# muyeon-jo/POI_recommendation_models

Measured on NVIDIA B200. Metric: fullrank_eval_users_per_sec, higher is better.
Workload: dtype f16+e5m2-corrections/f32-accum

## Files before the change

poi_recommendation_models_b200/csrc/nais_tc.cu:

```cuda
#include <cuda_fp16.h>
#include <cuda_fp8.h>

#include <type_traits>

#include "nais_common.cuh"
#include "umma.cuh"

namespace nais {

using namespace umma;

namespace tc {

constexpr int TM = 128;
constexpr int NBUF = 3;
constexpr int ACC_STRIDE = 160;
constexpr int TPC = 3;
constexpr int EPI_WARPS = 16;
constexpr int EPI_THREADS = EPI_WARPS * 32;
constexpr int ARRIVE_WARPS = 8;
constexpr int THREADS = (EPI_WARPS + 2) * 32;
constexpr int MAX_STAGES = 4;
constexpr int SORTN = 512;
constexpr int HMETA = 512;
// ... 366 lines not shown
  const int m = (int)(room < n ? (room < 0 ? 0 : room) : n);
  return m - m % hsplit;
}

struct MainArgs {
  NaisParams p;
  NaisCatalog cat;
  NaisUsers users;
  Geo g;
  int64_t poi_begin, poi_end;
  int k, exclude, groups;
  int groups_real;
  int64_t n_items;
  const unsigned char* hdr;
  const unsigned char* Pimg;
  const unsigned char* Bimg;
  unsigned long long* part_keys;
  float* all_scores;
  const float* score_in;
  int64_t max_chunks;
  int gate;
  const int* pass_flags;
  GeoMixArgs geo;
};

__device__ __forceinline__ void epi_bar() { asm volatile("bar.sync 1, 512;" ::: "memory"); }

__device__ __forceinline__ unsigned long long warp_sort_desc(unsigned long long v, int lane) {
#pragma unroll
  for (int k = 2; k <= 32; k <<= 1) {
#pragma unroll
    for (int j = k >> 1; j > 0; j >>= 1) {
      const unsigned long long o = __shfl_xor_sync(0xffffffffu, v, j);
      const bool desc = k == 32 || (lane & k) == 0, lower = (lane & j) == 0;
      v = (lower == desc) ? (v > o ? v : o) : (v < o ? v : o);
    }
  }
  return v;
}
__device__ __forceinline__ unsigned long long warp_fold_top32(unsigned long long a, unsigned long long b, int lane) {
  const unsigned long long br = __shfl_sync(0xffffffffu, b, 31 - lane);
  unsigned long long v = a > br ? a : br;
#pragma unroll
  for (int j = 16; j > 0; j >>= 1) {
    const unsigned long long o = __shfl_xor_sync(0xffffffffu, v, j);
    v = ((lane & j) == 0) ? (v > o ? v : o) : (v < o ? v : o);
  }
  return v;
}

template <bool kSinglePart, int kHch, int kFix, int kS = 64, bool kGeo = false>
__global__ void __launch_bounds__(THREADS, 1) fullrank_tc_kernel(const __grid_constant__ MainArgs A) {
  constexpr bool kPair = kFix == 5 || kFix == 6;
  constexpr bool kFastEpi = kFix == 1 || kFix == 2 || kPair;
  constexpr bool kD128 = kFix == 3;
  static_assert(!kGeo || kFix == 0 || kFix == 4, "geo mode lives in the run-time-shape epilogue");
  constexpr int kCombA = kGeo ? 4 : 3, kCombT = (kGeo && !kSinglePart) ? 2 : TPC;
  extern __shared__ __align__(128) unsigned char smem[];
  const Geo& g = A.g;
  unsigned char* sA = smem;
  unsigned char* sB = sA + g.tpc * g.a_tile;
  unsigned char* sE = sB + g.stages * g.stage_bytes;
  unsigned char* sZ = sE + NBUF * 2 * TM * 16;
  unsigned long long* keys = reinterpret_cast<unsigned long long*>(sZ + 4096);
  float* comb = kSinglePart ? reinterpret_cast<float*>(keys + SORTN) : reinterpret_cast<float*>(sE);
  int* hm_id = reinterpret_cast<int*>(reinterpret_cast<unsigned char*>(keys + SORTN) + (kSinglePart ? 3 * kCombA * TPC * TM * 4 : 0));
  float* hm_la = reinterpret_cast<float*>(hm_id + HMETA);
  float* hm_lo = hm_la + HMETA;
  float* xch = hm_lo + HMETA;
  uint64_t* bars = reinterpret_cast<uint64_t*>(xch + 6 * TM);
  uint64_t* a_full = bars + 0;
  uint64_t* a_empty = bars + 1;
  uint64_t* b_full = bars + 2;
  uint64_t* b_empty = bars + 2 + MAX_STAGES;
  uint64_t* e_full = bars + 2 + 2 * MAX_STAGES;
  uint64_t* acc_full = e_full + NBUF;
  uint64_t* acc_empty = acc_full + 2 * NBUF;
  uint32_t* tslot = reinterpret_cast<uint32_t*>(acc_empty + NBUF);
  float* hm_cos = reinterpret_cast<float*>(reinterpret_cast<unsigned char*>(bars) + 384);
// ... 36 lines not shown
    fence_barrier_init();
  }
  if (warp == EPI_WARPS) {
    if constexpr (kPair) tmem_alloc2(tslot, 512);
    else tmem_alloc(tslot, 512);
  }
  fence_proxy_async();
  tc_fence_before();
  __syncthreads();
  if constexpr (kPair) cluster_sync_all();
  tc_fence_after();
  const uint32_t tmem = *tslot;

  constexpr int tpc = kSinglePart ? TPC : (kFix == 4 ? 1 : 2);
  const int hsplit = kHch == 1 ? g.hsplit : 1;
  const int64_t cb0 = chunk_base(A.users.offsets, 0, kHch, hsplit);

  if (warp == EPI_WARPS + 1) {
    {
      uint32_t it_n = 0, bstep = 0;
      for (int64_t item = item0; item < A.n_items; item += item_step) {
        const int u = (int)(item / groups_it), grp = kPair ? 2 * (int)(item % groups_it) + (int)crank : (int)(item % groups_it);
        if (!user_in_pass(A.gate, sc.use_mix, (int)(A.users.offsets[u + 1] - A.users.offsets[u]))) continue;
        const uint32_t it = it_n++;
        const int64_t cbu = __shfl_sync(0xffffffffu, chunk_base(A.users.offsets, u, kHch, hsplit) - cb0, 0);
        const int nchunks = __shfl_sync(0xffffffffu, user_chunks(A.users.offsets, u, kHch, cb0, A.max_chunks, hsplit), 0);
        mbar_wait(a_empty, (it & 1) ^ 1);
        if (elect_one()) {
          mbar_expect_tx(a_full, (uint32_t)(tpc * g.a_tile));
          for (int t = 0; t < tpc; ++t)
            bulk_g2s(sA + (size_t)t * g.a_tile, A.Pimg + ((size_t)grp * tpc + t) * g.a_tile, (uint32_t)g.a_tile, a_full);
        }
        __syncwarp();
        const unsigned char* src = A.Bimg + (size_t)cbu * g.b_chunk + (kPair ? (size_t)crank * (g.b_chunk / 2) : 0);
        for (int c = 0; c < nchunks; ++c) {
          const int kp_t = kSinglePart ? 1 : g.kp;
          for (int pp = 0; pp < kp_t; ++pp, ++bstep) {
            const int st = bstep % g.stages;
            const uint32_t bytes = kPair ? (uint32_t)(g.b_chunk / 2) : (uint32_t)(pp == kp_t - 1 ? g.part_last_bytes : g.part_bytes);
            mbar_wait(&b_empty[st], ((bstep / g.stages) & 1) ^ 1);
            if (elect_one()) {
              mbar_expect_tx(&b_full[st], bytes);
              bulk_g2s(sB + (size_t)st * g.stage_bytes, src + (size_t)c * g.b_chunk + (size_t)pp * g.part_bytes, bytes, &b_full[st]);
            }
            __syncwarp();
          }
// ... 22 lines not shown
      };
      auto commit = [](uint64_t* bar) {
        if constexpr (kPair) mma2_commit_multicast(bar, 3);
        else mma_commit(bar);
      };
      const uint32_t zaddr = smem_u32(sZ);
      const uint32_t hi_word = (uint32_t)(smem_desc(0, 0, 128) >> 32);
      auto lo_of = [](uint32_t addr, uint32_t lbo) { return ((addr >> 4) & 0x3FFFu) | (((lbo >> 4) & 0x3FFFu) << 16); };
      auto mk = [&](uint32_t lo) { return ((uint64_t)hi_word << 32) | lo; };
      const uint32_t sa0 = smem_u32(sA), sb0 = smem_u32(sB), se0 = smem_u32(sE);
      const uint32_t A_hi = lo_of(sa0, kALbo);
      const uint32_t A_lo = lo_of(sa0 + kAPlane, kALbo);
      const uint32_t A_l8 = lo_of(sa0 + kAPlane + kAPlane / 2, kALbo);
      const uint32_t E_hi = lo_of(se0, zaddr - se0), E_lo = lo_of(se0 + TM * 16, zaddr - se0 - TM * 16);
      constexpr uint32_t kEz = kExtBuf - (kExtBuf << 16), kBz = kStage - (kStage << 16);
      const uint32_t E_mx = lo_of(se0, TM * 16);
      const uint32_t B_hi = lo_of(sb0, kBLbo);
      const uint32_t Bx_hi = lo_of(sb0 + kKx * kBLbo, zaddr - (sb0 + kKx * kBLbo));
      const uint32_t Bx_lo = lo_of(sb0 + (2 * kKx + 1) * kBLbo, zaddr - (sb0 + (2 * kKx + 1) * kBLbo));
      uint32_t it_n = 0, cc = 0, st = 0, stph = 0;
      for (int64_t item = item0; item < A.n_items; item += item_step) {
        const int u = (int)(item / groups_it);
        if (!user_in_pass(A.gate, sc.use_mix, (int)(A.users.offsets[u + 1] - A.users.offsets[u]))) continue;
        const uint32_t it = it_n++;
        const int nchunks = __shfl_sync(0xffffffffu, user_chunks(A.users.offsets, u, kHch, cb0, A.max_chunks, hsplit), 0);
        mbar_wait(a_full, it & 1);
        if constexpr (kPair) {
          if (crank != 0) {
            if (elect_one()) mbar_arrive_cluster(a_full_peer, 0);
            __syncwarp();
            for (int c = 0; c < nchunks; ++c) {
              mbar_wait(&b_full[st], stph);
              if (elect_one()) mbar_arrive_cluster(&b_full_peer[st], 0);
              __syncwarp();
              st = (st + 1u) % kStages;
              stph ^= (st == 0);
            }
            continue;
          }
          mbar_wait_cluster(a_full_peer, it & 1);
        }
        for (int c = 0; c < nchunks; ++c, ++cc) {
          mbar_wait(&b_full[st], stph);
          if constexpr (kPair) mbar_wait_cluster(&b_full_peer[st], stph);
          const uint32_t cph = cc & 1u;
          const uint32_t bh = B_hi + st * kStage;
// ... 164 lines not shown
    const int npos = sc.npos, hid = g.hid;
    constexpr int hch = kHch;
    const int ncols = hch == 2 ? hid : hid / 2;
    const int col0 = hs * ncols;
    const int kidx0 = hch == 2 ? 0 : col0 + (hsplit == 2 ? egrp * hid : 0);
    auto div_tpc = [&](int x) { return x / tpc; };
    uint32_t n0 = 0;
    uint32_t phbits = 0;
    uint32_t fph = 0;
    const float c_a2 = sc.inv_sigma * 1.4426950408889634f, inv_sAe = 1.f / sc.sAe;
    const float bd0s = bd0 - log2f(sc.sAe), bd1s = bd1 - log2f(sc.sAe);
    const int nposb = npos >> 4, nposm = npos & 15;
    const float* sgn_mixed = xch;

    auto arrive_mma = [&](uint64_t* bar) {
      if constexpr (kPair) mbar_arrive_cluster(bar, 0);
      else mbar_arrive(bar);
    };
    for (int64_t item = item0; item < A.n_items; item += item_step) {
      const int u = (int)(item / groups_it), grp = kPair ? 2 * (int)(item % groups_it) + (int)crank : (int)(item % groups_it);
      const int64_t hb = A.users.offsets[u];
      const int H = (int)(A.users.offsets[u + 1] - hb);
      if (!user_in_pass(A.gate, sc.use_mix, H)) continue;
      const int nchunks = user_chunks(A.users.offsets, u, hch, cb0, A.max_chunks, hsplit);
      const int nsteps = nchunks * tpc;
      epi_bar();
      for (int i = tid; i < H && i < HMETA; i += EPI_THREADS) {
        hm_id[i] = __ldg(A.users.items + hb + i);
        hm_la[i] = (geo || kGeo) ? __ldg(A.users.coords + 2 * (hb + i)) : 0.f;
        hm_lo[i] = (geo || kGeo) ? __ldg(A.users.coords + 2 * (hb + i) + 1) : 0.f;
        if constexpr (!kFastEpi)
          if (g.km || kGeo) hm_cos[i] = cosf((A.cat.center_lat + hm_la[i]) * 0.017453292519943295f);
      }
      float clat[TPC], clon[TPC], ccos[TPC], sumE[TPC], sumES[TPC], sumL[TPC];
      int64_t jid[TPC];
      bool excl[TPC];
#pragma unroll
      for (int t = 0; t < TPC; ++t) {
        jid[t] = t < tpc ? A.poi_begin + ((int64_t)grp * tpc + t) * TM + r : A.poi_end;
        const bool v = jid[t] < A.poi_end;
        clat[t] = (v && (geo || kGeo)) ? __ldg(A.cat.coords + 2 * (jid[t] - A.cat.row_base)) : 0.f;
        clon[t] = (v && (geo || kGeo)) ? __ldg(A.cat.coords + 2 * (jid[t] - A.cat.row_base) + 1) : 0.f;
        ccos[t] = 1.f;
        if constexpr (!kFastEpi)
          if (g.km || kGeo) ccos[t] = cosf((A.cat.center_lat + clat[t]) * 0.017453292519943295f);
        sumE[t] = 0.f;
// ... 93 lines not shown
            tmem_wait_ld16(va);
            tmem_wait_ld16(vb);
            if constexpr (kS == 64) {
              blk(va, 0);
              tmem_ld16(tb_main + t * ACC_STRIDE + 32, va);
              blk(vb, 1);
              tmem_ld16(tb_main + t * ACC_STRIDE + 48, vb);
              tmem_wait_ld16(va);
              tmem_wait_ld16(vb);
            }
            tc_fence_before();
            __syncwarp();
            if (lane == 0) arrive_mma(&acc_empty[t]);
            if constexpr (kS == 64) {
              blk(va, 2);
              blk(vb, 3);
            } else {
              blk(va, 0);
              blk(vb, 1);
            }
            const float asum = ((p0 + p1) + (p2 + p3)) - ((q0 + q1) + (q2 + q3));
            const float S = __uint_as_float(aux[0]) * sc.inv_s;
            const float a2 = (__uint_as_float(aux[1]) + asum) * c_a2;
            const bool same = hist_id == jt[t];
            const float e = (hvalid && !same) ? ex2_approx(a2) : 0.f;
            sumE[t] += e;
            sumES[t] = fmaf(e, S, sumES[t]);
            excl[t] = excl[t] || (hvalid && same);
          }
          fph ^= 1u;
        }
      } else {
        auto produce = [&](int m) {
          const int pc = div_tpc(m), pt = m - pc * tpc;
          const uint32_t pbuf = (n0 + (uint32_t)m) % NBUF;
          const int h = hch == 2 ? 2 * pc + hs : pc / hsplit;
          float g0 = 0.f, g1 = 0.f;
          if (g.lanes && h < H && (hch == 2 || hs == 0)) {
            float hla, hlo;
            if (h < HMETA) {
              hla = hm_la[h];
              hlo = hm_lo[h];
            } else {
              hla = __ldg(A.users.coords + 2 * (hb + h));
              hlo = __ldg(A.users.coords + 2 * (hb + h) + 1);
            }
            const float ct_la = pt == 0 ? clat[0] : (pt == 1 ? clat[1] : clat[2]);
            const float ct_lo = pt == 0 ? clon[0] : (pt == 1 ? clon[1] : clon[2]);
            const float l0 = fabsf(ct_la - hla), l1 = fabsf(ct_lo - hlo);
            const float z0 = fmaf(l1, w01, fmaf(l0, w00, bd0)), z1 = fmaf(l1, w11, fmaf(l0, w10, bd1));
            g0 = __fdividef(sc.sAe, 1.f + exp2f(z0));
// ... 118 lines not shown
                } else {
                  hla = __ldg(A.users.coords + 2 * (hb + h));
                  hlo = __ldg(A.users.coords + 2 * (hb + h) + 1);
                  hcs = cosf((A.cat.center_lat + hla) * 0.017453292519943295f);
                }
                const float cla = t == 0 ? clat[0] : (t == 1 ? clat[1] : clat[2]), clo = t == 0 ? clon[0] : (t == 1 ? clon[1] : clon[2]);
                const float ccs = t == 0 ? ccos[0] : (t == 1 ? ccos[1] : ccos[2]);
                const float km = dist_km_f(cla, clo, hla, hlo, ccs, hcs);
                a_km = fmaf(km, ckm, a);
              }
              const float e = g.km ? expf(a_km) : __expf(a);
              if (t == 0) { sumE[0] += e; sumES[0] = fmaf(e, S, sumES[0]); }
              else if (t == 1) { sumE[1] += e; sumES[1] = fmaf(e, S, sumES[1]); }
              else { sumE[2] += e; sumES[2] = fmaf(e, S, sumES[2]); }
            } else {
              if (t == 0) excl[0] = true;
              else if (t == 1) excl[1] = true;
              else excl[2] = true;
            }
          }
        }
        n0 += (uint32_t)nsteps;
      }
      const int part = egrp * 2 + hs;
      const bool small_k = A.k <= 32;
      unsigned long long kreg[TPC];
      if (!kSinglePart) epi_bar();
      if (part != 0) {
#pragma unroll
        for (int t2 = 0; t2 < kCombT; ++t2) {
          comb[((part - 1) * kCombA + 0) * kCombT * TM + t2 * TM + r] = sumE[t2];
          comb[((part - 1) * kCombA + 1) * kCombT * TM + t2 * TM + r] = sumES[t2];
          comb[((part - 1) * kCombA + 2) * kCombT * TM + t2 * TM + r] = excl[t2] ? 1.f : 0.f;
          if constexpr (kGeo) comb[((part - 1) * kCombA + 3) * kCombT * TM + t2 * TM + r] = sumL[t2];
        }
      }
      epi_bar();
      if (part == 0) {
#pragma unroll
        for (int t2 = 0; t2 < TPC; ++t2) {
          float E = sumE[t2], ES = sumES[t2], Lg = sumL[t2];
          bool ex = excl[t2];
          if (t2 < kCombT) {
#pragma unroll
            for (int q = 0; q < 3; ++q) {
              E += comb[(q * kCombA + 0) * kCombT * TM + t2 * TM + r];
// ... 42 lines not shown
              if (desc ? (x < y) : (x > y)) {
                keys[i] = y;
                keys[ixj] = x;
              }
            }
          }
          epi_bar();
        }
      }
      if (grp < A.groups_real)
        for (int i = tid; i < A.k; i += EPI_THREADS) A.part_keys[((size_t)u * A.groups_real + grp) * A.k + i] = keys[i];
    }
  }
  tc_fence_before();
  __syncthreads();
  if constexpr (kPair) cluster_sync_all();
  if (warp == EPI_WARPS) {
    if constexpr (kPair) tmem_dealloc2(tmem, 512);
    else tmem_dealloc(tmem, 512);
  }
}


}

int launch_topk_merge(const unsigned long long* in_keys, const float* in_score, const int32_t* in_id, int n_users,
                      int n_lists, int k, float* out_score, int32_t* out_id, cudaStream_t stream);
int launch_topk_merge_keys_multi(const unsigned long long* keys, unsigned long long* scratch, int64_t user_stride, int64_t list_stride,
                                 int n_users, int n_lists, int k, unsigned long long* out_keys, float* out_score, int32_t* out_id,
                                 cudaStream_t stream);
int merge_scratch_lists(int n_lists, int k);

static inline size_t al256(size_t x) { return (x + 255) / 256 * 256; }

struct PlanLayout {
  tc::Geo g, gs;
  bool two_pass;
  bool pair;
  tc::Geo gp, gsp;
  int groups, n_tiles_pad;
  size_t hdr, pimg, pimg2, total;
};

static bool plan_layout(const NaisParams& p, int64_t poi_begin, int64_t poi_end, int precision, PlanLayout& L) {
  const int prec = precision & NAIS_PREC_MASK;
  if (!tc::make_geo(p, prec, L.g)) return false;
// ... 54 lines not shown

bool tc_supported(const NaisParams& p, int precision) {
  for (int bi = 0; bi < p.n_branch; ++bi) {
    tc::Geo g;
    if (!tc::make_geo(branch_view(p, bi), precision & NAIS_PREC_MASK, g)) return false;
  }
  return true;
}

static size_t plan_bytes_1(const NaisParams& p, int64_t poi_begin, int64_t poi_end, int precision) {
  PlanLayout L;
  return plan_layout(p, poi_begin, poi_end, precision, L) ? L.total : 0;
}
size_t fullrank_tc_plan_bytes(const NaisParams& p, int64_t poi_begin, int64_t poi_end, int precision) {
  size_t total = 0;
  for (int bi = 0; bi < p.n_branch; ++bi) {
    const size_t b = plan_bytes_1(branch_view(p, bi), poi_begin, poi_end, precision);
    if (!b) return 0;
    total += b;
  }
  return total;
}

static size_t call_workspace_bytes_1(const NaisParams& p, int n_users, int64_t nnz, int64_t poi_begin, int64_t poi_end, int k,
                                     int precision) {
  PlanLayout L;
  if (!plan_layout(p, poi_begin, poi_end, precision, L)) return 0;
  const int64_t max_chunks = (L.g.hch == 2 ? (nnz + n_users) / 2 : nnz * L.g.hsplit) + 2;
  return 256 + al256((size_t)max_chunks * L.g.b_chunk) + call_keys_bytes(n_users, L.groups, k) + call_scratch_bytes(n_users, L.groups, k);
}
size_t fullrank_tc_call_workspace_bytes(const NaisParams& p, int n_users, int64_t nnz, int64_t poi_begin, int64_t poi_end, int k,
                                        int precision) {
  size_t most = 0;
  for (int bi = 0; bi < p.n_branch; ++bi) {
    const size_t b = call_workspace_bytes_1(branch_view(p, bi), n_users, nnz, poi_begin, poi_end, k, precision);
    if (!b) return 0;
    most = b > most ? b : most;
  }
  return most + branch_scores_bytes(p, n_users, poi_begin, poi_end);
}

size_t fullrank_tc_workspace_bytes(const NaisParams& p, int n_users, int64_t nnz, int64_t poi_begin, int64_t poi_end, int k,
                                   int precision) {
  const size_t a = fullrank_tc_plan_bytes(p, poi_begin, poi_end, precision);
  const size_t b = fullrank_tc_call_workspace_bytes(p, n_users, nnz, poi_begin, poi_end, k, precision);
  return (a && b) ? a + b + 1024 + (size_t)n_users * 8 : 0;
}

static int check_arch(int& sms) {
  int dev = 0, major = 0;
  cudaGetDevice(&dev);
  cudaDeviceGetAttribute(&major, cudaDevAttrComputeCapabilityMajor, dev);
  if (major != 10) return NAIS_ERR_ARCH;
  sms = 148;
  cudaDeviceGetAttribute(&sms, cudaDevAttrMultiProcessorCount, dev);
  return 0;
}

// ... 50 lines not shown
  return 0;
}

typedef void (*MainKernel)(const tc::MainArgs);

static MainKernel pick_kernel(const tc::Geo& gg, bool generic) {
  const bool s64 = gg.D == 64 && gg.hid == 64 && gg.nrow == 144, s32 = gg.D == 32 && gg.hid == 32 && gg.nrow == 80;
  if (gg.km) generic = true;
  const int fix = ((s64 || s32) && gg.kp == 1 && gg.hch == 2 && gg.stages == 2 && !generic) ? (gg.mix ? 2 : (gg.split ? 1 : 0)) : 0;
  if (gg.pair) return gg.mix ? tc::fullrank_tc_kernel<true, 2, 6, 64> : tc::fullrank_tc_kernel<true, 2, 5, 64>;
  if (gg.kp == 1) {
    if (gg.hch != 2) return tc::fullrank_tc_kernel<true, 1, 0>;
    if (fix == 2) return s64 ? tc::fullrank_tc_kernel<true, 2, 2, 64> : tc::fullrank_tc_kernel<true, 2, 2, 32>;
    if (fix == 1) return s64 ? tc::fullrank_tc_kernel<true, 2, 1, 64> : tc::fullrank_tc_kernel<true, 2, 1, 32>;
    return tc::fullrank_tc_kernel<true, 2, 0>;
  }
  if (gg.tpc == 1) return gg.hch == 2 ? tc::fullrank_tc_kernel<false, 2, 4> : tc::fullrank_tc_kernel<false, 1, 4>;
  if (gg.hch == 2) return tc::fullrank_tc_kernel<false, 2, 0>;
  if (gg.D == 128 && gg.hid == 128 && gg.kp == 4 && gg.nrow == 144 && gg.stages == 3 && (gg.mix || gg.split) && !generic)
    return tc::fullrank_tc_kernel<false, 1, 3>;
  return tc::fullrank_tc_kernel<false, 1, 0>;
}

static MainKernel pick_geo_kernel(const tc::Geo& gg) {
  if (gg.kp == 1) return gg.hch == 2 ? tc::fullrank_tc_kernel<true, 2, 0, 64, true> : tc::fullrank_tc_kernel<true, 1, 0, 64, true>;
  if (gg.tpc == 1) return gg.hch == 2 ? tc::fullrank_tc_kernel<false, 2, 4, 64, true> : tc::fullrank_tc_kernel<false, 1, 4, 64, true>;
  return gg.hch == 2 ? tc::fullrank_tc_kernel<false, 2, 0, 64, true> : tc::fullrank_tc_kernel<false, 1, 0, 64, true>;
}
static int geo_extra_smem(const tc::Geo& gg) { return (gg.kp == 1 ? 3 * tc::TPC * tc::TM * 4 : 0) + (gg.km ? 0 : tc::HMETA * 4); }

static int run_1(const NaisParams& p, const NaisCatalog& cat, const NaisUsers& users, int64_t poi_begin, int64_t poi_end, int k,
                 int exclude, int precision, const void* plan, size_t plan_bytes, unsigned long long* out_keys, float* out_score,
                 int32_t* out_id, float* all_scores, const float* score_in, bool merge, void* ws, size_t ws_bytes, cudaStream_t stream,
                 const GeoMixArgs* geo = nullptr) {
  if (users.n_users == 0 || poi_end <= poi_begin) return 0;
  int sms;
  int rc = check_arch(sms);
  if (rc) return rc;
  PlanLayout L;
  if (!plan_layout(p, poi_begin, poi_end, precision, L)) return NAIS_ERR_SHAPE;
  if (!plan || plan_bytes < L.total) return NAIS_ERR_WORKSPACE;
  const unsigned char* pbase = reinterpret_cast<const unsigned char*>(plan);
  const unsigned char* hdr = pbase + L.hdr;
  const size_t keys_bytes = call_keys_bytes(users.n_users, L.groups, k), scratch_bytes = call_scratch_bytes(users.n_users, L.groups, k);
  if (ws_bytes < 256 + keys_bytes + scratch_bytes + (size_t)L.g.b_chunk) return NAIS_ERR_WORKSPACE;
  unsigned char* base = reinterpret_cast<unsigned char*>(ws);
  int* pass_flags = reinterpret_cast<int*>(base);
  const size_t bimg_bytes = (ws_bytes - 256 - keys_bytes - scratch_bytes) / 256 * 256;
  unsigned char* bimg = base + 256;
  unsigned long long* keys = reinterpret_cast<unsigned long long*>(base + 256 + bimg_bytes);
  unsigned long long* scratch = reinterpret_cast<unsigned long long*>(base + 256 + bimg_bytes + keys_bytes);
  const int64_t max_chunks = (int64_t)(bimg_bytes / L.g.b_chunk);
// ... 16 lines not shown
    if (st == 0) {
      cudaLaunchConfig_t cfg = {};
      cfg.gridDim = dim3(2);
      cfg.blockDim = dim3(tc::THREADS);
      cfg.dynamicSmemBytes = L.gp.smem_bytes;
      cudaLaunchAttribute at[1];
      at[0].id = cudaLaunchAttributeClusterDimension;
      at[0].val.clusterDim.x = 2;
      at[0].val.clusterDim.y = 1;
      at[0].val.clusterDim.z = 1;
      cfg.attrs = at;
      cfg.numAttrs = 1;
      MainKernel kp = pick_kernel(L.gp, false);
      int n = 0;
      const bool ok = cudaFuncSetAttribute(kp, cudaFuncAttributeMaxDynamicSharedMemorySize, L.gp.smem_bytes) == cudaSuccess &&
                      cudaOccupancyMaxActiveClusters(&n, kp, &cfg) == cudaSuccess && n >= 1;
      if (!ok) cudaGetLastError();
      st = ok ? 1 : -1;
    }
    use_pair = st == 1;
  }
  const tc::Geo& g1 = use_pair ? L.gp : L.g;
  const tc::Geo& g2 = use_pair ? L.gsp : L.gs;
  {
    dim3 grid(users.n_users, 64);
    tc::pack_users_kernel<<<grid, 256, 0, stream>>>(p, users, g1, g2, L.two_pass ? 1 : 0, hdr, bimg, max_chunks, pass_flags,
                                                   bad_index_flag());
    NAIS_COUNT_LAUNCH(1);
  }
  auto run = [&](const tc::Geo& gg, const unsigned char* pimg, int gate) -> int {
    tc::MainArgs A;
    A.p = p;
    A.cat = cat;
    A.users = users;
    A.g = gg;
    A.poi_begin = poi_begin;
    A.poi_end = poi_end;
    A.k = k;
    A.exclude = exclude;
    A.groups = gg.pair ? (L.groups + 1) / 2 * 2 : L.groups;
    A.groups_real = L.groups;
    A.n_items = (int64_t)users.n_users * (gg.pair ? A.groups / 2 : A.groups);
    A.hdr = hdr;
    A.Pimg = pimg;
    A.Bimg = bimg;
    A.part_keys = keys;
    A.all_scores = all_scores;
    A.score_in = score_in;
    A.max_chunks = max_chunks;
    A.gate = gate;
    A.pass_flags = pass_flags;
    A.geo = geo ? *geo : GeoMixArgs{};
    MainKernel kern = geo ? pick_geo_kernel(gg) : pick_kernel(gg, generic);
    const int smem = gg.smem_bytes + (geo ? geo_extra_smem(gg) : 0);
    cudaError_t e2 = cudaFuncSetAttribute(kern, cudaFuncAttributeMaxDynamicSharedMemorySize, smem);
    if (e2 != cudaSuccess) return (int)e2;
    if (gg.pair) {
      const int pairs = (int)(A.n_items < sms / 2 ? A.n_items : sms / 2);
      cudaLaunchConfig_t cfg = {};
      cfg.gridDim = dim3(2 * pairs);
      cfg.blockDim = dim3(tc::THREADS);
      cfg.dynamicSmemBytes = gg.smem_bytes;
      cfg.stream = stream;
      cudaLaunchAttribute at[1];
      at[0].id = cudaLaunchAttributeClusterDimension;
      at[0].val.clusterDim.x = 2;
      at[0].val.clusterDim.y = 1;
      at[0].val.clusterDim.z = 1;
      cfg.attrs = at;
      cfg.numAttrs = 1;
      e2 = cudaLaunchKernelEx(&cfg, kern, A);
      NAIS_COUNT_LAUNCH(1);
      return e2 == cudaSuccess ? 0 : (int)e2;
    }
    const int grid = (int)(A.n_items < sms ? A.n_items : sms);
    kern<<<grid, tc::THREADS, smem, stream>>>(A);
    NAIS_COUNT_LAUNCH(1);
    e2 = cudaGetLastError();
    return e2 == cudaSuccess ? 0 : (int)e2;
  };
  if (L.two_pass) {
    rc = run(g1, pbase + L.pimg, 1);
    if (rc) return rc;
    rc = run(g2, pbase + L.pimg2, 0);
  } else {
    rc = run(g1, pbase + L.pimg, -1);
  }
  if (rc || !merge) return rc;
  return launch_topk_merge_keys_multi(keys, scratch, (int64_t)L.groups * k, k, users.n_users, L.groups, k, out_keys, out_score, out_id,
                                      stream);
}

int fullrank_tc_run(const NaisParams& p, const NaisCatalog& cat, const NaisUsers& users, int64_t poi_begin, int64_t poi_end, int k,
                    int exclude, int precision, const void* plan, size_t plan_bytes, unsigned long long* out_keys, float* out_score,
                    int32_t* out_id, float* all_scores, void* ws, size_t ws_bytes, cudaStream_t stream, const GeoMixArgs* geo) {
  if (users.n_users == 0 || poi_end <= poi_begin) return 0;
  if (p.n_branch == 1)
    return run_1(p, cat, users, poi_begin, poi_end, k, exclude, precision, plan, plan_bytes, out_keys, out_score, out_id, all_scores,
                 nullptr, true, ws, ws_bytes, stream, geo);
  const size_t sbytes = branch_scores_bytes(p, users.n_users, poi_begin, poi_end);
  if (!plan || ws_bytes < sbytes + 512) return NAIS_ERR_WORKSPACE;
  float* sbuf = reinterpret_cast<float*>(ws);
// ... 32 lines not shown
```

Baseline: 12490.

## Deduplicate history items across users and reuse per-item attention tiles

```diff
diff --git a/poi_recommendation_models_b200/csrc/nais_tc.cu b/poi_recommendation_models_b200/csrc/nais_tc.cu
--- a/poi_recommendation_models_b200/csrc/nais_tc.cu
+++ b/poi_recommendation_models_b200/csrc/nais_tc.cu
@@ -1,5 +1,8 @@
 #include <cuda_fp16.h>
 #include <cuda_fp8.h>
+
+#include <cub/device/device_radix_sort.cuh>
+#include <cub/device/device_scan.cuh>
 
 #include <type_traits>
 
@@ -412,6 +415,8 @@
   int gate;
   const int* pass_flags;
   GeoMixArgs geo;
+  float2* es;
+  int64_t es_ld;
 };
 
 __device__ __forceinline__ void epi_bar() { asm volatile("bar.sync 1, 512;" ::: "memory"); }
@@ -439,12 +444,13 @@
   return v;
 }
 
-template <bool kSinglePart, int kHch, int kFix, int kS = 64, bool kGeo = false>
+template <bool kSinglePart, int kHch, int kFix, int kS = 64, bool kGeo = false, bool kStore = false>
 __global__ void __launch_bounds__(THREADS, 1) fullrank_tc_kernel(const __grid_constant__ MainArgs A) {
   constexpr bool kPair = kFix == 5 || kFix == 6;
   constexpr bool kFastEpi = kFix == 1 || kFix == 2 || kPair;
   constexpr bool kD128 = kFix == 3;
   static_assert(!kGeo || kFix == 0 || kFix == 4, "geo mode lives in the run-time-shape epilogue");
+  static_assert(!kStore || (kFastEpi && kS == 64), "store mode lives in the D = hid = 64 specialised epilogue");
   constexpr int kCombA = kGeo ? 4 : 3, kCombT = (kGeo && !kSinglePart) ? 2 : TPC;
   extern __shared__ __align__(128) unsigned char smem[];
   const Geo& g = A.g;
@@ -527,6 +533,8 @@
       for (int64_t item = item0; item < A.n_items; item += item_step) {
         const int u = (int)(item / groups_it), grp = kPair ? 2 * (int)(item % groups_it) + (int)crank : (int)(item % groups_it);
         if (!user_in_pass(A.gate, sc.use_mix, (int)(A.users.offsets[u + 1] - A.users.offsets[u]))) continue;
+        if constexpr (kStore)
+          if (A.users.offsets[u + 1] == A.users.offsets[u]) continue;
         const uint32_t it = it_n++;
         const int64_t cbu = __shfl_sync(0xffffffffu, chunk_base(A.users.offsets, u, kHch, hsplit) - cb0, 0);
         const int nchunks = __shfl_sync(0xffffffffu, user_chunks(A.users.offsets, u, kHch, cb0, A.max_chunks, hsplit), 0);
@@ -595,6 +603,8 @@
       for (int64_t item = item0; item < A.n_items; item += item_step) {
         const int u = (int)(item / groups_it);
         if (!user_in_pass(A.gate, sc.use_mix, (int)(A.users.offsets[u + 1] - A.users.offsets[u]))) continue;
+        if constexpr (kStore)
+          if (A.users.offsets[u + 1] == A.users.offsets[u]) continue;
         const uint32_t it = it_n++;
         const int nchunks = __shfl_sync(0xffffffffu, user_chunks(A.users.offsets, u, kHch, cb0, A.max_chunks, hsplit), 0);
         mbar_wait(a_full, it & 1);
@@ -805,6 +815,8 @@
       const int64_t hb = A.users.offsets[u];
       const int H = (int)(A.users.offsets[u + 1] - hb);
       if (!user_in_pass(A.gate, sc.use_mix, H)) continue;
+      if constexpr (kStore)
+        if (H == 0) continue;
       const int nchunks = user_chunks(A.users.offsets, u, hch, cb0, A.max_chunks, hsplit);
       const int nsteps = nchunks * tpc;
       epi_bar();
@@ -944,11 +956,15 @@
             const float asum = ((p0 + p1) + (p2 + p3)) - ((q0 + q1) + (q2 + q3));
             const float S = __uint_as_float(aux[0]) * sc.inv_s;
             const float a2 = (__uint_as_float(aux[1]) + asum) * c_a2;
-            const bool same = hist_id == jt[t];
-            const float e = (hvalid && !same) ? ex2_approx(a2) : 0.f;
-            sumE[t] += e;
-            sumES[t] = fmaf(e, S, sumES[t]);
-            excl[t] = excl[t] || (hvalid && same);
+            if constexpr (kStore) {
+              if (hvalid && jt[t] >= 0) A.es[(size_t)(hb + h) * A.es_ld + (jid[t] - A.poi_begin)] = make_float2(ex2_approx(a2), S);
+            } else {
+              const bool same = hist_id == jt[t];
+              const float e = (hvalid && !same) ? ex2_approx(a2) : 0.f;
+              sumE[t] += e;
+              sumES[t] = fmaf(e, S, sumES[t]);
+              excl[t] = excl[t] || (hvalid && same);
+            }
           }
           fph ^= 1u;
         }
@@ -1113,6 +1129,7 @@
         }
         n0 += (uint32_t)nsteps;
       }
+      if constexpr (kStore) continue;
       const int part = egrp * 2 + hs;
       const bool small_k = A.k <= 32;
       unsigned long long kreg[TPC];
@@ -1201,6 +1218,143 @@
 }
 
 
+__global__ void dedup_keys_kernel(NaisParams p, NaisCatalog cat, NaisUsers users, int gate, const unsigned char* hdr, int cmp_region,
+                                  int cmp_coords, int bits, int64_t n_cap, unsigned long long* keys, int* vals) {
+  const Scales* sc = reinterpret_cast<const Scales*>(hdr + 64);
+  const int u = blockIdx.x;
+  const int64_t e0 = users.offsets[0], hb = users.offsets[u], he = users.offsets[u + 1];
+  if (!user_in_pass(gate, sc->use_mix, (int)(he - hb))) return;
+  for (int64_t e = hb + threadIdx.x; e < he && e - e0 < n_cap; e += blockDim.x) {
+    const int item = __ldg(users.items + e);
+    const int64_t jl = (int64_t)item - cat.row_base;
+    bool own = item < 0 || item >= p.item_num;
+    if (!own && (cmp_region || cmp_coords)) {
+      if (jl < 0 || jl >= cat.n_rows) {
+        own = true;
+      } else {
+        if (cmp_region && __ldg(users.region + e) != __ldg(cat.region + jl)) own = true;
+        if (cmp_coords && (__float_as_uint(__ldg(users.coords + 2 * e)) != __float_as_uint(__ldg(cat.coords + 2 * jl)) ||
+                           __float_as_uint(__ldg(users.coords + 2 * e + 1)) != __float_as_uint(__ldg(cat.coords + 2 * jl + 1))))
+          own = true;
+      }
+    }
+    const unsigned long long id = own ? (unsigned long long)p.item_num + (unsigned long long)(e - e0) : (unsigned long long)item;
+    keys[e - e0] = ((unsigned long long)((e - hb) & 1) << bits) | id;
+    vals[e - e0] = (int)(e - e0);
+  }
+}
+
+__global__ void dedup_runs_kernel(const unsigned long long* keys, int64_t n, int bits, unsigned long long* flag) {
+  const unsigned long long mask = (2ull << bits) - 1;
+  for (int64_t i = blockIdx.x * (int64_t)blockDim.x + threadIdx.x; i < n; i += (int64_t)gridDim.x * blockDim.x) {
+    const unsigned long long k = keys[i] & mask;
+    const bool start = k != mask && (i == 0 || (keys[i - 1] & mask) != k);
+    flag[i] = start ? ((k >> bits) ? (1ull << 32) : 1ull) : 0ull;
+  }
+}
+
+__device__ __forceinline__ int dedup_row(unsigned long long scan, int slot) {
+  return slot ? 2 * (int)((scan >> 32) - 1) + 1 : 2 * (int)((scan & 0xffffffffull) - 1);
+}
+__global__ void dedup_rows_kernel(NaisUsers users, const unsigned long long* keys, const int* vals, const unsigned long long* scan,
+                                  int64_t n, int bits, int* entry_row, int* row_item, int* row_region, float2* row_coords) {
+  const unsigned long long mask = (2ull << bits) - 1;
+  const int64_t e0 = users.offsets[0];
+  for (int64_t i = blockIdx.x * (int64_t)blockDim.x + threadIdx.x; i < n; i += (int64_t)gridDim.x * blockDim.x) {
+    const unsigned long long k = keys[i] & mask;
+    if (k == mask) continue;
+    const int r = dedup_row(scan[i], (int)(k >> bits));
+    const int el = vals[i];
+    entry_row[el] = r;
+    if (i == 0 || (keys[i - 1] & mask) != k) {
+      row_item[r] = __ldg(users.items + e0 + el);
+      if (row_region) row_region[r] = __ldg(users.region + e0 + el);
+      if (row_coords) row_coords[r] = __ldg(reinterpret_cast<const float2*>(users.coords) + e0 + el);
+    }
+  }
+}
+
+__global__ void dedup_finish_kernel(const unsigned long long* scan, int64_t n, int64_t R, int V, int* row_item, int* row_region,
+                                    float2* row_coords, int64_t* voffs) {
+  const unsigned long long s = n > 0 ? scan[n - 1] : 0ull;
+  const int64_t x0 = (int64_t)(s & 0xffffffffull), x1 = (int64_t)(s >> 32), X = 2 * (x0 > x1 ? x0 : x1);
+  for (int64_t i = blockIdx.x * (int64_t)blockDim.x + threadIdx.x; i < R || i <= V; i += (int64_t)gridDim.x * blockDim.x) {
+    if (i < X && row_item[i] < 0) {
+      row_item[i] = row_item[i ^ 1];
+      if (row_region) row_region[i] = row_region[i ^ 1];
+      if (row_coords) row_coords[i] = row_coords[i ^ 1];
+    }
+    if (i <= V) voffs[i] = 128 * i < X ? 128 * i : X;
+  }
+}
+
+constexpr int RED_THREADS = TPC * TM;
+__global__ void __launch_bounds__(RED_THREADS) dedup_reduce_kernel(NaisUsers users, float beta, const unsigned char* hdr, int gate,
+                                                                   const int* entry_row, int64_t n_cap, const float2* es, int64_t es_ld,
+                                                                   int64_t slab_begin, int64_t poi_end, int group0, int groups_real,
+                                                                   int k, int exclude, unsigned long long* part_keys) {
+  __shared__ unsigned long long keys[SORTN];
+  const Scales* sc = reinterpret_cast<const Scales*>(hdr + 64);
+  const int u = blockIdx.x, grp = group0 + (int)blockIdx.y, tid = threadIdx.x;
+  const int64_t hb = users.offsets[u];
+  const int H = (int)(users.offsets[u + 1] - hb);
+  if (grp >= groups_real || !user_in_pass(gate, sc->use_mix, H)) return;
+  const int64_t el0 = hb - users.offsets[0];
+  const int Hc = (int)(el0 >= n_cap ? 0 : (n_cap - el0 < H ? n_cap - el0 : H));
+  const int c = (int)blockIdx.y * RED_THREADS + tid;
+  const int64_t j = slab_begin + c;
+  const bool valid = j < poi_end;
+  float E[4] = {0.f, 0.f, 0.f, 0.f}, ES[4] = {0.f, 0.f, 0.f, 0.f};
+  bool ex = false;
+  if (valid) {
+    const float2* col = es + c;
+    const int* er = entry_row + el0;
+    const int* it = users.items + hb;
+    const int jj = (int)j;
+    for (int h = 0; h < Hc; h += 8) {
+      float2 v[8];
+      int id[8];
+#pragma unroll
+      for (int q = 0; q < 8; ++q) {
+        v[q] = h + q < Hc ? __ldg(col + (size_t)__ldg(er + h + q) * es_ld) : make_float2(0.f, 0.f);
+        id[q] = h + q < Hc ? __ldg(it + h + q) : -1;
+      }
+#pragma unroll
+      for (int q = 0; q < 8; ++q) {
+        if (h + q < Hc) {
+          const bool same = id[q] == jj;
+          const float e = same ? 0.f : v[q].x;
+          E[q & 3] += e;
+          ES[q & 3] = fmaf(e, v[q].y, ES[q & 3]);
+          ex = ex || same;
+        }
+      }
+    }
+  }
+  const float Et = ((E[0] + E[1]) + E[2]) + E[3], ESt = ((ES[0] + ES[1]) + ES[2]) + ES[3];
+  const float score = ESt / powf(Et, beta);
+  keys[tid] = (valid && !(exclude && ex)) ? make_key(score, (int)j) : 0ull;
+  for (int i = RED_THREADS + tid; i < SORTN; i += RED_THREADS) keys[i] = 0ull;
+  __syncthreads();
+  for (int kk = 2; kk <= SORTN; kk <<= 1) {
+    for (int jj = kk >> 1; jj > 0; jj >>= 1) {
+      for (int i = tid; i < SORTN; i += RED_THREADS) {
+        const int ixj = i ^ jj;
+        if (ixj > i) {
+          const unsigned long long x = keys[i], y = keys[ixj];
+          const bool desc = (i & kk) == 0;
+          if (desc ? (x < y) : (x > y)) {
+            keys[i] = y;
+            keys[ixj] = x;
+          }
+        }
+      }
+      __syncthreads();
+    }
+  }
+  for (int i = tid; i < k; i += RED_THREADS) part_keys[((size_t)u * groups_real + grp) * k + i] = keys[i];
+}
+
 }
 
 int launch_topk_merge(const unsigned long long* in_keys, const float* in_score, const int32_t* in_id, int n_users,
@@ -1301,18 +1455,97 @@
   return total;
 }
 
+static size_t old_workspace_bytes_1(const PlanLayout& L, int n_users, int64_t nnz, int k) {
+  const int64_t max_chunks = (L.g.hch == 2 ? (nnz + n_users) / 2 : nnz * L.g.hsplit) + 2;
+  return 256 + al256((size_t)max_chunks * L.g.b_chunk) + call_keys_bytes(n_users, L.groups, k) + call_scratch_bytes(n_users, L.groups, k);
+}
+
+constexpr double kDedupKappa = 2.0;
+constexpr int64_t kDedupSlabUnit = 2 * tc::TPC * tc::TM;
+constexpr size_t kDedupEsBudget = size_t(1) << 30;
+
+static bool dedup_shape(const PlanLayout& L, int precision) {
+  auto fix64 = [](const tc::Geo& q) {
+    return q.D == 64 && q.hid == 64 && q.nrow == 144 && q.kp == 1 && q.hch == 2 && q.stages == 2 && !q.km && (q.mix || q.split);
+  };
+  return !(precision & NAIS_PREC_FLAG_GENERIC) && fix64(L.g) && fix64(L.gs);
+}
+static bool dedup_selected(const NaisParams& p, const PlanLayout& L, int precision, int64_t nnz) {
+  return dedup_shape(L, precision) && (double)nnz >= kDedupKappa * 2.0 * (double)p.item_num;
+}
+
+struct DedupLayout {
+  int64_t n_cap, R, max_chunks, slab;
+  int V, bits;
+  size_t img, es, erow, kin, kout, vin, vout, scan, ritem, rreg, rcoord, voffs, cub, cub_bytes, total;
+};
+static bool dedup_layout(const PlanLayout& L, int n_users, int64_t n_cap, int k, DedupLayout& D) {
+  D.n_cap = n_cap < 0 ? 0 : n_cap;
+  D.R = D.n_cap + n_users + 2;
+  D.V = (int)((D.R + 127) / 128);
+  D.max_chunks = (D.R + D.V) / 2 + 2;
+  D.bits = 1;
+  while ((1ll << D.bits) <= D.n_cap + (1ll << 31)) ++D.bits;
+  const int64_t range_pad = (int64_t)L.n_tiles_pad * tc::TM;
+  const int64_t width = (range_pad + kDedupSlabUnit - 1) / kDedupSlabUnit * kDedupSlabUnit;
+  const double full = (double)D.R * (double)width * 8.0, unit = (double)D.R * (double)kDedupSlabUnit * 8.0;
+  const double es_bytes = full <= (double)kDedupEsBudget ? full : (unit > (double)kDedupEsBudget ? unit : (double)kDedupEsBudget);
+  int64_t slab = (int64_t)(es_bytes / ((double)D.R * 8.0)) / kDedupSlabUnit * kDedupSlabUnit;
+  D.slab = slab < kDedupSlabUnit ? kDedupSlabUnit : (slab > width ? width : slab);
+  size_t cb_sort = 0, cb_scan = 0;
+  const int ni = (int)(D.n_cap > 0x7fffffff ? 0x7fffffff : D.n_cap);
+  cub::DoubleBuffer<unsigned long long> kb(nullptr, nullptr);
+  cub::DoubleBuffer<int> vb(nullptr, nullptr);
+  cub::DeviceRadixSort::SortPairs(nullptr, cb_sort, kb, vb, ni, 0, D.bits + 1);
+  cub::DeviceScan::InclusiveSum(nullptr, cb_scan, (const unsigned long long*)nullptr, (unsigned long long*)nullptr, ni);
+  D.cub_bytes = cb_sort > cb_scan ? cb_sort : cb_scan;
+  size_t o = 256 + call_keys_bytes(n_users, L.groups, k) + call_scratch_bytes(n_users, L.groups, k);
+  auto put = [&](size_t& at, size_t bytes) { at = o; o += al256(bytes); };
+  put(D.img, (size_t)D.max_chunks * L.g.b_chunk);
+  put(D.es, (size_t)D.R * (size_t)D.slab * 8);
+  put(D.erow, (size_t)D.n_cap * 4);
+  put(D.kin, (size_t)D.n_cap * 8);
+  put(D.kout, (size_t)D.n_cap * 8);
+  put(D.vin, (size_t)D.n_cap * 4);
+  put(D.vout, (size_t)D.n_cap * 4);
+  put(D.scan, (size_t)D.n_cap * 8);
+  put(D.ritem, (size_t)D.R * 4);
+  put(D.rreg, (size_t)D.R * 4);
+  put(D.rcoord, (size_t)D.R * 8);
+  put(D.voffs, (size_t)(D.V + 1) * 8);
+  put(D.cub, D.cub_bytes + 256);
+  D.total = o;
+  return true;
+}
+static size_t dedup_workspace_bytes_1(const PlanLayout& L, int n_users, int64_t nnz, int k) {
+  DedupLayout D;
+  dedup_layout(L, n_users, nnz, k, D);
+  const size_t old = old_workspace_bytes_1(L, n_users, nnz, k);
+  return D.total > old ? D.total : old;
+}
+static int64_t dedup_nnz_of_workspace(const PlanLayout& L, int n_users, int k, size_t ws_bytes) {
+  int64_t lo = 0, hi = int64_t(1) << 40;
+  if (dedup_workspace_bytes_1(L, n_users, 0, k) > ws_bytes) return -1;
+  while (lo < hi) {
+    const int64_t mid = lo + (hi - lo + 1) / 2;
+    if (dedup_workspace_bytes_1(L, n_users, mid, k) <= ws_bytes) lo = mid;
+    else hi = mid - 1;
+  }
+  return lo;
+}
+
 static size_t call_workspace_bytes_1(const NaisParams& p, int n_users, int64_t nnz, int64_t poi_begin, int64_t poi_end, int k,
-                                     int precision) {
+                                     int precision, bool one_branch) {
   PlanLayout L;
   if (!plan_layout(p, poi_begin, poi_end, precision, L)) return 0;
-  const int64_t max_chunks = (L.g.hch == 2 ? (nnz + n_users) / 2 : nnz * L.g.hsplit) + 2;
-  return 256 + al256((size_t)max_chunks * L.g.b_chunk) + call_keys_bytes(n_users, L.groups, k) + call_scratch_bytes(n_users, L.groups, k);
+  if (one_branch && dedup_selected(p, L, precision, nnz)) return dedup_workspace_bytes_1(L, n_users, nnz, k);
+  return old_workspace_bytes_1(L, n_users, nnz, k);
 }
 size_t fullrank_tc_call_workspace_bytes(const NaisParams& p, int n_users, int64_t nnz, int64_t poi_begin, int64_t poi_end, int k,
                                         int precision) {
   size_t most = 0;
   for (int bi = 0; bi < p.n_branch; ++bi) {
-    const size_t b = call_workspace_bytes_1(branch_view(p, bi), n_users, nnz, poi_begin, poi_end, k, precision);
+    const size_t b = call_workspace_bytes_1(branch_view(p, bi), n_users, nnz, poi_begin, poi_end, k, precision, p.n_branch == 1);
     if (!b) return 0;
     most = b > most ? b : most;
   }
@@ -1409,12 +1642,113 @@
   return tc::fullrank_tc_kernel<false, 1, 0>;
 }
 
+static MainKernel pick_store_kernel(const tc::Geo& gg) {
+  if (gg.pair) return gg.mix ? tc::fullrank_tc_kernel<true, 2, 6, 64, false, true> : tc::fullrank_tc_kernel<true, 2, 5, 64, false, true>;
+  return gg.mix ? tc::fullrank_tc_kernel<true, 2, 2, 64, false, true> : tc::fullrank_tc_kernel<true, 2, 1, 64, false, true>;
+}
+
 static MainKernel pick_geo_kernel(const tc::Geo& gg) {
   if (gg.kp == 1) return gg.hch == 2 ? tc::fullrank_tc_kernel<true, 2, 0, 64, true> : tc::fullrank_tc_kernel<true, 1, 0, 64, true>;
   if (gg.tpc == 1) return gg.hch == 2 ? tc::fullrank_tc_kernel<false, 2, 4, 64, true> : tc::fullrank_tc_kernel<false, 1, 4, 64, true>;
   return gg.hch == 2 ? tc::fullrank_tc_kernel<false, 2, 0, 64, true> : tc::fullrank_tc_kernel<false, 1, 0, 64, true>;
 }
 static int geo_extra_smem(const tc::Geo& gg) { return (gg.kp == 1 ? 3 * tc::TPC * tc::TM * 4 : 0) + (gg.km ? 0 : tc::HMETA * 4); }
+
+template <class LaunchMain>
+static int run_dedup(const NaisParams& p, const NaisCatalog& cat, const NaisUsers& users, int64_t poi_begin, int64_t poi_end, int k,
+                     int exclude, const PlanLayout& L, const tc::Geo& g1, const tc::Geo& g2, const unsigned char* pbase, int64_t n_cap,
+                     unsigned char* base, size_t ws_bytes, unsigned long long* keys, cudaStream_t stream, LaunchMain& launch_main) {
+  DedupLayout D;
+  dedup_layout(L, users.n_users, n_cap, k, D);
+  if (D.total > ws_bytes) return NAIS_ERR_WORKSPACE;
+  const unsigned char* hdr = pbase + L.hdr;
+  unsigned char* img = base + D.img;
+  float2* es = reinterpret_cast<float2*>(base + D.es);
+  int* erow = reinterpret_cast<int*>(base + D.erow);
+  unsigned long long* kin = reinterpret_cast<unsigned long long*>(base + D.kin);
+  unsigned long long* kout = reinterpret_cast<unsigned long long*>(base + D.kout);
+  int* vin = reinterpret_cast<int*>(base + D.vin);
+  int* vout = reinterpret_cast<int*>(base + D.vout);
+  unsigned long long* scan = reinterpret_cast<unsigned long long*>(base + D.scan);
+  int* ritem = reinterpret_cast<int*>(base + D.ritem);
+  int* rreg = users.region ? reinterpret_cast<int*>(base + D.rreg) : nullptr;
+  float2* rcoord = users.coords ? reinterpret_cast<float2*>(base + D.rcoord) : nullptr;
+  int64_t* voffs = reinterpret_cast<int64_t*>(base + D.voffs);
+  const NaisUsers vu{voffs, ritem, rreg, reinterpret_cast<const float*>(rcoord), D.V};
+  const int cmp_region = p.branch[0].w_reg > 0 ? 1 : 0, cmp_coords = L.g.lanes ? 1 : 0;
+  const int64_t range = poi_end - poi_begin;
+  const int ethreads = 256;
+  const int eblocks = (int)((D.n_cap + ethreads - 1) / ethreads < 4096 ? (D.n_cap + ethreads - 1) / ethreads : 4096);
+  const int rblocks = (int)(((D.R > D.V ? D.R : D.V + 1) + ethreads - 1) / ethreads < 4096 ? ((D.R > D.V ? D.R : D.V + 1) + ethreads - 1) / ethreads : 4096);
+  cudaError_t e;
+  auto pass = [&](const tc::Geo& gg, const unsigned char* pimg, int gate) -> int {
+    if ((e = cudaMemsetAsync(kin, 0xFF, (size_t)D.n_cap * 8, stream)) != cudaSuccess) return (int)e;
+    if ((e = cudaMemsetAsync(ritem, 0xFF, (size_t)D.R * 4, stream)) != cudaSuccess) return (int)e;
+    tc::dedup_keys_kernel<<<users.n_users, 128, 0, stream>>>(p, cat, users, gate, hdr, cmp_region, cmp_coords, D.bits, D.n_cap, kin, vin);
+    NAIS_COUNT_LAUNCH(1);
+    cub::DoubleBuffer<unsigned long long> kb(kin, kout);
+    cub::DoubleBuffer<int> vb(vin, vout);
+    size_t cb = D.cub_bytes;
+    if ((e = cub::DeviceRadixSort::SortPairs(base + D.cub, cb, kb, vb, (int)D.n_cap, 0, D.bits + 1, stream)) != cudaSuccess) return (int)e;
+    NAIS_COUNT_LAUNCH(1);
+    unsigned long long* flag = kb.Alternate();
+    tc::dedup_runs_kernel<<<eblocks, ethreads, 0, stream>>>(kb.Current(), D.n_cap, D.bits, flag);
+    NAIS_COUNT_LAUNCH(1);
+    cb = D.cub_bytes;
+    if ((e = cub::DeviceScan::InclusiveSum(base + D.cub, cb, flag, scan, (int)D.n_cap, stream)) != cudaSuccess) return (int)e;
+    NAIS_COUNT_LAUNCH(1);
+    tc::dedup_rows_kernel<<<eblocks, ethreads, 0, stream>>>(users, kb.Current(), vb.Current(), scan, D.n_cap, D.bits, erow, ritem, rreg,
+                                                            rcoord);
+    NAIS_COUNT_LAUNCH(1);
+    tc::dedup_finish_kernel<<<rblocks, ethreads, 0, stream>>>(scan, D.n_cap, D.R, D.V, ritem, rreg, rcoord, voffs);
+    NAIS_COUNT_LAUNCH(1);
+    tc::pack_users_kernel<<<dim3(D.V, 64), 256, 0, stream>>>(p, vu, gg, gg, 0, hdr, img, D.max_chunks, nullptr, bad_index_flag());
+    NAIS_COUNT_LAUNCH(1);
+    const MainKernel kern = pick_store_kernel(gg);
+    for (int64_t s0 = 0; s0 < range; s0 += D.slab) {
+      const int64_t s1 = s0 + D.slab < range ? s0 + D.slab : range;
+      const int groups = (int)(((s1 - s0 + tc::TM - 1) / tc::TM + gg.tpc - 1) / gg.tpc);
+      tc::MainArgs A;
+      A.p = p;
+      A.cat = cat;
+      A.users = vu;
+      A.g = gg;
+      A.poi_begin = poi_begin + s0;
+      A.poi_end = poi_begin + s1;
+      A.k = k;
+      A.exclude = exclude;
+      A.groups = gg.pair ? (groups + 1) / 2 * 2 : groups;
+      A.groups_real = groups;
+      A.n_items = (int64_t)D.V * (gg.pair ? A.groups / 2 : A.groups);
+      A.hdr = hdr;
+      A.Pimg = pimg + (size_t)(s0 / tc::TM) * gg.a_tile;
+      A.Bimg = img;
+      A.part_keys = nullptr;
+      A.all_scores = nullptr;
+      A.score_in = nullptr;
+      A.max_chunks = D.max_chunks;
+      A.gate = -1;
+      A.pass_flags = nullptr;
+      A.geo = GeoMixArgs{};
+      A.es = es;
+      A.es_ld = D.slab;
+      int rc = launch_main(kern, A, gg.smem_bytes);
+      if (rc) return rc;
+      tc::dedup_reduce_kernel<<<dim3(users.n_users, groups), tc::RED_THREADS, 0, stream>>>(
+          users, p.beta, hdr, gate, erow, D.n_cap, es, D.slab, poi_begin + s0, poi_end, (int)(s0 / (tc::TPC * tc::TM)), L.groups, k,
+          exclude, keys);
+      NAIS_COUNT_LAUNCH(1);
+      if ((e = cudaGetLastError()) != cudaSuccess) return (int)e;
+    }
+    return 0;
+  };
+  if (L.two_pass) {
+    const int rc = pass(g1, pbase + L.pimg, 1);
+    if (rc) return rc;
+    return pass(g2, pbase + L.pimg2, 0);
+  }
+  return pass(g1, pbase + L.pimg, -1);
+}
 
 static int run_1(const NaisParams& p, const NaisCatalog& cat, const NaisUsers& users, int64_t poi_begin, int64_t poi_end, int k,
                  int exclude, int precision, const void* plan, size_t plan_bytes, unsigned long long* out_keys, float* out_score,
@@ -1477,6 +1811,44 @@
   }
   const tc::Geo& g1 = use_pair ? L.gp : L.g;
   const tc::Geo& g2 = use_pair ? L.gsp : L.gs;
+  auto launch_main = [&](MainKernel kern, const tc::MainArgs& A, int smem) -> int {
+    cudaError_t e2 = cudaFuncSetAttribute(kern, cudaFuncAttributeMaxDynamicSharedMemorySize, smem);
+    if (e2 != cudaSuccess) return (int)e2;
+    if (A.g.pair) {
+      const int pairs = (int)(A.n_items < sms / 2 ? A.n_items : sms / 2);
+      cudaLaunchConfig_t cfg = {};
+      cfg.gridDim = dim3(2 * pairs);
+      cfg.blockDim = dim3(tc::THREADS);
+      cfg.dynamicSmemBytes = smem;
+      cfg.stream = stream;
+      cudaLaunchAttribute at[1];
+      at[0].id = cudaLaunchAttributeClusterDimension;
+      at[0].val.clusterDim.x = 2;
+      at[0].val.clusterDim.y = 1;
+      at[0].val.clusterDim.z = 1;
+      cfg.attrs = at;
+      cfg.numAttrs = 1;
+      e2 = cudaLaunchKernelEx(&cfg, kern, A);
+      NAIS_COUNT_LAUNCH(1);
+      return e2 == cudaSuccess ? 0 : (int)e2;
+    }
+    const int grid = (int)(A.n_items < sms ? A.n_items : sms);
+    kern<<<grid, tc::THREADS, smem, stream>>>(A);
+    NAIS_COUNT_LAUNCH(1);
+    e2 = cudaGetLastError();
+    return e2 == cudaSuccess ? 0 : (int)e2;
+  };
+  if (merge && !all_scores && !score_in && !geo && dedup_shape(L, precision)) {
+    const int64_t n_cap = dedup_nnz_of_workspace(L, users.n_users, k, ws_bytes);
+    if (n_cap >= 0 && (double)n_cap >= kDedupKappa * 2.0 * (double)p.item_num) {
+      unsigned long long* dkeys = reinterpret_cast<unsigned long long*>(base + 256);
+      unsigned long long* dscratch = reinterpret_cast<unsigned long long*>(base + 256 + keys_bytes);
+      rc = run_dedup(p, cat, users, poi_begin, poi_end, k, exclude, L, g1, g2, pbase, n_cap, base, ws_bytes, dkeys, stream, launch_main);
+      if (rc) return rc;
+      return launch_topk_merge_keys_multi(dkeys, dscratch, (int64_t)L.groups * k, k, users.n_users, L.groups, k, out_keys, out_score,
+                                          out_id, stream);
+    }
+  }
   {
     dim3 grid(users.n_users, 64);
     tc::pack_users_kernel<<<grid, 256, 0, stream>>>(p, users, g1, g2, L.two_pass ? 1 : 0, hdr, bimg, max_chunks, pass_flags,
@@ -1506,33 +1878,10 @@
     A.gate = gate;
     A.pass_flags = pass_flags;
     A.geo = geo ? *geo : GeoMixArgs{};
+    A.es = nullptr;
+    A.es_ld = 0;
     MainKernel kern = geo ? pick_geo_kernel(gg) : pick_kernel(gg, generic);
-    const int smem = gg.smem_bytes + (geo ? geo_extra_smem(gg) : 0);
-    cudaError_t e2 = cudaFuncSetAttribute(kern, cudaFuncAttributeMaxDynamicSharedMemorySize, smem);
-    if (e2 != cudaSuccess) return (int)e2;
-    if (gg.pair) {
-      const int pairs = (int)(A.n_items < sms / 2 ? A.n_items : sms / 2);
-      cudaLaunchConfig_t cfg = {};
-      cfg.gridDim = dim3(2 * pairs);
-      cfg.blockDim = dim3(tc::THREADS);
-      cfg.dynamicSmemBytes = gg.smem_bytes;
-      cfg.stream = stream;
-      cudaLaunchAttribute at[1];
-      at[0].id = cudaLaunchAttributeClusterDimension;
-      at[0].val.clusterDim.x = 2;
-      at[0].val.clusterDim.y = 1;
-      at[0].val.clusterDim.z = 1;
-      cfg.attrs = at;
-      cfg.numAttrs = 1;
-      e2 = cudaLaunchKernelEx(&cfg, kern, A);
-      NAIS_COUNT_LAUNCH(1);
-      return e2 == cudaSuccess ? 0 : (int)e2;
-    }
-    const int grid = (int)(A.n_items < sms ? A.n_items : sms);
-    kern<<<grid, tc::THREADS, smem, stream>>>(A);
-    NAIS_COUNT_LAUNCH(1);
-    e2 = cudaGetLastError();
-    return e2 == cudaSuccess ? 0 : (int)e2;
+    return launch_main(kern, A, gg.smem_bytes + (geo ? geo_extra_smem(gg) : 0));
   };
   if (L.two_pass) {
     rc = run(g1, pbase + L.pimg, 1);
```

Measured after the change: 31490, median of 6. +152.1%, better.
